# SowpatiLab/ribbit

Hardware: AMD Instinct MI355X
Metric: Gbases/s scanned (m=2..100) (higher is better)
Workload: dtype u32 bit planes

## Files before the change

### ribbit_amd/csrc/api_core.cpp

```cpp
#include "api_internal.h"

#include <sys/mman.h>

namespace rbapi {

thread_local std::string g_last_error;

int fail(int code, const char *fmt, ...) {
    char buf[512];
    va_list ap;
    va_start(ap, fmt);
    vsnprintf(buf, sizeof buf, fmt, ap);
    va_end(ap);
    g_last_error = buf;
    return code;
}


namespace {
constexpr size_t PINNED_HUGE_FROM = (size_t)64 << 20;
std::mutex g_mapped_mu;
std::vector<std::pair<void *, size_t>> g_mapped;
}

// ... 69 lines not shown
int is_gfx950(int device) {
    hipDeviceProp_t prop;
    if (hipGetDeviceProperties(&prop, device) != hipSuccess) return 0;
    return std::strncmp(prop.gcnArchName, "gfx950", 6) == 0;
}

int pack_loaded_ascii(RibbitHandle *h, const uint8_t *dev_ascii, int64_t length) {
    if (h->pair_pending) return fail(RIBBIT_E_STATE, "a perfect scan is in flight on this handle: call ribbit_hip_scan_perfect_end first");
    if (h->copy_pending) { const int rcw = perfect_wait(h); if (rcw) return rcw; }
    h->loaded = false;
    h->dev_ascii_src = dev_ascii;
    h->rec = RibbitHandle::RecordState{};
    if (h->xa_copy_pending) { (void)hipEventSynchronize(h->ev_xa); h->xa_copy_pending = false; }
    h->length = length;
    const int64_t nwords = length / 32 + 1;
    h->ntiles = (nwords + rb::TILE_WORDS - 1) / rb::TILE_WORDS;
    h->tail_words = h->max_shift / 32 + rb::TAIL_SLACK_WORDS;
    h->total_words = rb::LEAD_WORDS + h->ntiles * rb::TILE_WORDS + h->tail_words;
    int rc;
    if ((rc = h->d_hi.ensure((size_t)h->total_words))) return rc;
    if ((rc = h->d_lo.ensure((size_t)h->total_words))) return rc;
    if ((rc = h->d_brk.ensure((size_t)h->total_words))) return rc;
    if (h->timing) HIP_TRY(hipEventRecord(h->timers.begin[RIBBIT_TIME_PACK], h->stream));
    if ((rc = h->pb.d_counters.ensure(rb::EV_COUNTER_WORDS))) return rc;
    rb::launch_pack(dev_ascii, length, h->d_hi.p, h->d_lo.p, h->d_brk.p, h->total_words, h->pb.d_counters.p, rb::EV_COUNTER_WORDS, h->stream);
    h->counters_clean = true;
    HIP_TRY(hipGetLastError());
    if (h->timing) HIP_TRY(hipEventRecord(h->timers.end[RIBBIT_TIME_PACK], h->stream));
    h->timers.have[RIBBIT_TIME_PACK] = h->timing;
    h->lists.perfect.clear(); h->lists.subst.clear(); h->lists.anchored.clear();
    h->lists.range_count = nullptr;
    h->lists.guard_hits = 0;
    h->lists.plane_words = nullptr; h->lists.plane_stride = 0; h->lists.plane_lo = 0; h->lists.plane_hi = -1;
    h->lists.length = length;
    h->lists.min_motif = h->params.min_motif;
    h->lists.max_motif = h->params.max_motif;
    h->lists.min_shift = h->min_shift;
    h->loaded = true;
    return RIBBIT_OK;
}

int ensure_host_planes(RibbitHandle *h) {
    if (h->rec.host_planes_valid) return RIBBIT_OK;
    int rc;
    if ((rc = bind_device(h))) return rc;
    const size_t n = (size_t)(h->ntiles * rb::TILE_WORDS + h->tail_words);
    h->host.resize(h->length, n);
    HIP_TRY(hipMemcpyAsync(h->host.hi.data(), h->d_hi.p + rb::LEAD_WORDS, n * sizeof(uint32_t), hipMemcpyDeviceToHost, h->stream));
    HIP_TRY(hipMemcpyAsync(h->host.lo.data(), h->d_lo.p + rb::LEAD_WORDS, n * sizeof(uint32_t), hipMemcpyDeviceToHost, h->stream));
// ... 283 lines not shown
    } else if (what == RIBBIT_TIME_ANCHORED_PLANES || what == RIBBIT_TIME_ANCHORED_WINDOW) {
        if (!anchored.have_timing || !h->planes_timing_valid) return fail(RIBBIT_E_STATE, "the anchored stage has not run as two kernels on this handle");
        from = what == RIBBIT_TIME_ANCHORED_PLANES ? anchored.ev_begin : h->ev_planes;
        to = what == RIBBIT_TIME_ANCHORED_PLANES ? h->ev_planes : anchored.ev_end;
        last = anchored.ev_end;
    } else {
        if (what < 0 || what > RIBBIT_TIME_ANCHORED_WINDOW) return fail(RIBBIT_E_ARG, "what must be 0..9");
        if (!h->timers.have[what]) return fail(RIBBIT_E_STATE, "no timing recorded yet");
        from = h->timers.begin[what]; to = last = h->timers.end[what];
    }
    float f = 0.f;
    HIP_TRY(hipEventSynchronize(last));
    HIP_TRY(hipEventElapsedTime(&f, from, to));
    *ms = f;
    return RIBBIT_OK;
}); }

int ribbit_hip_debug_stream_read(RibbitHandle *h, int64_t nbytes, int64_t *bytes_read) { return guarded("the stream read", [&]() -> int {
    if (!h || !bytes_read) return fail(RIBBIT_E_ARG, "null argument");
    if (!h->loaded) return fail(RIBBIT_E_STATE, "no record loaded");
    int rc;
    if ((rc = bind_device(h))) return rc;
    if ((rc = h->pb.d_counters.ensure(rb::EV_COUNTER_WORDS))) return rc;
    const uint32_t *src = h->d_events.p ? (const uint32_t *)h->d_events.p : h->d_hi.p;
    const int64_t avail = h->d_events.p ? (int64_t)h->d_events.cap * 8 : h->total_words * 4;
    const int64_t n = std::max<int64_t>(0, std::min(nbytes, avail)) / 4;
    rb::launch_calib_stream_read(src, n, h->pb.d_counters.p + rb::EV_SUMMARY + 8, h->stream);
    HIP_TRY(hipGetLastError());
    HIP_TRY(hipStreamSynchronize(h->stream));
    *bytes_read = n * 4;
    return RIBBIT_OK;
}); }

int64_t ribbit_hip_last_event_count(const RibbitHandle *h) { return h ? h->last_event_count : 0; }

}
```

### ribbit_amd/csrc/api_events.cpp

```cpp
#include "api_internal.h"

namespace rbapi {

int pair_prepare(RibbitHandle *h, PairBufs &pb, int64_t length, int64_t own_lo, int64_t own_hi, int64_t pos_offset, rb::PairLaunch &pr) {
    int rc;
    pr.m_lo = (uint32_t)h->params.min_motif;
    pr.nm = (uint32_t)(h->params.max_motif - h->params.min_motif + 1);
    pr.tile_bases = (uint32_t)rb::TILE_BASES;
    pr.ntile = (uint32_t)(length / rb::TILE_BASES + 1);
    pr.own_lo = own_lo; pr.own_hi = own_hi; pr.pos_offset = pos_offset;
    const size_t entries = (size_t)pr.nm * pr.ntile;
    if (entries > 0xfffffff0u) return fail(RIBBIT_E_ARG, "record too long for %u motif sizes", pr.nm);
    if ((rc = pb.d_counters.ensure(rb::EV_COUNTER_WORDS)) || (rc = pb.d_pair_status.ensure(rb::PAIR_STATUS_WORDS)) ||
        (rc = pb.d_pair_table.ensure(entries)) || (rc = pb.d_run_base.ensure(entries)) || (rc = pb.d_pair_partial.ensure(entries / 1024 + 2)) ||
        (rc = pb.d_halves.ensure(2 * (size_t)pr.nm)))
        return rc;
    if (!pb.h_pub.p) {
        if ((rc = pb.h_pub.ensure(rb::EV_SHARDS + rb::PAIR_STATUS_WORDS))) return rc;
        HIP_TRY(hipHostGetDevicePointer((void **)&pb.h_pub_dev, pb.h_pub.p, 0));
    }
    return RIBBIT_OK;
}

size_t first_event_cap(const RibbitHandle *h, size_t per_base_x4) {
    if (h->debug_first_cap) return h->debug_first_cap;
    return std::max(std::max<size_t>((size_t)1 << 20, (size_t)h->length * per_base_x4 / 4), h->d_events.cap);
}

static size_t round_event_cap(size_t cap) { return std::min<size_t>((cap + rb::EV_SHARDS - 1) / rb::EV_SHARDS * rb::EV_SHARDS, 0xffffff00u); }

int grow_event_cap(int attempt, uint32_t worst, size_t *cap) {
    const size_t need = (size_t)worst * rb::EV_SHARDS;
    if (attempt == 2 || round_event_cap(need) < need) return fail(RIBBIT_E_OVERFLOW, "event buffer overflow: fullest region needs %u events", worst);
    *cap = ((size_t)worst + 1024) * rb::EV_SHARDS;
    return RIBBIT_OK;
}

int event_room(RibbitHandle *h, size_t *cap, rb::PairLaunch *pr) {
    int rc;
    *cap = round_event_cap(*cap);
    if ((rc = h->d_events.ensure(*cap)) || (rc = h->d_dense.ensure(*cap))) return rc;
    if (pr) pr->region_cap = (uint32_t)(*cap / rb::EV_SHARDS);
    return RIBBIT_OK;
}

int zero_counters(RibbitHandle *h, bool even_if_clean) {
    if (even_if_clean || !h->counters_clean) HIP_TRY(hipMemsetAsync(h->pb.d_counters.p, 0, rb::EV_COUNTER_WORDS * sizeof(uint32_t), h->stream));
    h->counters_clean = false;
    return RIBBIT_OK;
}

rb::PerfectLaunch scan_launch_args(const RibbitHandle *h, size_t cap, int kernel) {
    rb::PerfectLaunch pp;
    pp.m_lo = h->params.min_motif;
    pp.m_hi = h->params.max_motif;
    pp.ev_cap = (uint32_t)cap;
    pp.motifs_per_block = h->debug_split[kernel];
    return pp;
}

int enqueue_pairing(PairBufs &pb, const rb::PairLaunch &pr, const uint64_t *d_events, uint64_t *d_dense, size_t cap, hipStream_t stream) {
    HIP_TRY(rb::launch_pair_runs(d_events, pb.d_counters.p, pr, pb.d_pair_table.p, pb.d_run_base.p, pb.d_pair_partial.p,
                                 d_dense, (uint32_t)(cap / 2), pb.d_halves.p, (uint32_t)(2 * (size_t)pr.nm), pb.d_pair_status.p, stream));
    rb::launch_pair_publish(pb.d_counters.p, pb.d_pair_status.p, pb.h_pub_dev, stream);
    HIP_TRY(hipGetLastError());
    return RIBBIT_OK;
}

Published read_published(const PairBufs &pb) {
    Published pub;
    for (int t = 0; t < rb::EV_SHARDS; ++t) { pub.worst = std::max(pub.worst, pb.h_pub.p[t]); pub.produced += pb.h_pub.p[t]; }
    return pub;
}

int pairing_verdict(const PairBufs &pb, uint64_t produced, const char *noun, size_t *n, size_t *n_halves) {
    const uint32_t *status = pb.h_pub.p + rb::EV_SHARDS, flags = status[rb::PAIR_FLAGS];
    if (flags) {
        const std::string s = noun;
        return fail(RIBBIT_E_INTERNAL, "%s pairing failed (flags 0x%x):%s%s%s%s%s", noun, flags,
                    flags & rb::PAIR_BAD_EVENT ? " malformed event;" : "", flags & rb::PAIR_DUP_CHUNK ? " duplicate event chunk;" : "",
                    flags & rb::PAIR_NOT_ALTERNATING ? (" " + s + " starts and ends do not alternate;").c_str() : "",
                    flags & rb::PAIR_UNTERMINATED ? (" unterminated " + s + ";").c_str() : "", flags & rb::PAIR_NO_ROOM ? (" " + s + " buffer too small;").c_str() : "");
    }
    *n = status[rb::PAIR_TOTAL];
    if ((uint64_t)*n * 2 != produced) return fail(RIBBIT_E_INTERNAL, "%llu events but %zu %ss", (unsigned long long)produced, *n, noun);
    *n_halves = status[rb::PAIR_HALVES];
    return RIBBIT_OK;
}

int collect_perfect_events(RibbitHandle *h) {
    int rc;
    if ((rc = bind_device(h))) return rc;
    if ((rc = h->pb.d_counters.ensure(rb::EV_COUNTER_WORDS))) return rc;
    if ((rc = h->h_counters.ensure(rb::EV_COUNTER_WORDS))) return rc;
    size_t cap = first_event_cap(h, 1);
    uint32_t produced = 0;
    for (int attempt = 0;; ++attempt) {
        if ((rc = event_room(h, &cap, nullptr))) return rc;
        HIP_TRY(hipEventRecord(h->timers.begin[RIBBIT_TIME_GPU], h->stream));
        if ((rc = zero_counters(h, true))) return rc;
        const rb::PerfectLaunch pp = scan_launch_args(h, cap, RIBBIT_SCAN_PERFECT);
        HIP_TRY(hipEventRecord(h->timers.begin[RIBBIT_TIME_SCAN], h->stream));
        h->rec.last_split[RIBBIT_SCAN_PERFECT] = rb::launch_scan_perfect(h->planes(), pp, h->d_events.p, h->pb.d_counters.p, h->stream);
        HIP_TRY(hipGetLastError());
        HIP_TRY(hipEventRecord(h->timers.end[RIBBIT_TIME_SCAN], h->stream));
        rb::launch_compact_events(h->d_events.p, pp.ev_cap, h->pb.d_counters.p, h->d_dense.p, h->stream);
        HIP_TRY(hipGetLastError());
        HIP_TRY(hipMemcpyAsync(h->h_counters.p, h->pb.d_counters.p, rb::EV_COUNTER_WORDS * sizeof(uint32_t), hipMemcpyDeviceToHost, h->stream));
        HIP_TRY(hipStreamSynchronize(h->stream));
        produced = h->h_counters.p[rb::EV_SUMMARY];
        if (!h->h_counters.p[rb::EV_SUMMARY + 1]) break;
        uint32_t worst = 0;
        for (int t = 0; t < rb::EV_SHARDS; ++t) worst = std::max(worst, h->h_counters.p[t * rb::EV_COUNTER_STRIDE]);
        if ((rc = grow_event_cap(attempt, worst, &cap))) return rc;
    }
    h->last_event_count = produced;
    if ((rc = h->h_events.ensure(std::max<size_t>(produced, 1)))) return rc;
    const uint32_t m_lo = (uint32_t)h->params.min_motif;
    const size_t nm = (size_t)(h->params.max_motif - h->params.min_motif + 1);
    const size_t ntile = (size_t)(h->length / rb::TILE_BASES + 1);
    if (nm * ntile > 0xfffffff0u) return fail(RIBBIT_E_ARG, "record too long for %zu motif sizes", nm);
    if ((rc = h->pb.d_pair_table.ensure(nm * ntile))) return rc;
    if ((rc = h->pb.d_pair_status.ensure(rb::PAIR_STATUS_WORDS))) return rc;
    HIP_TRY(rb::launch_chunk_table(h->d_dense.p, h->pb.d_counters.p, m_lo, (uint32_t)nm, (uint32_t)ntile, (uint32_t)rb::TILE_BASES, h->pb.d_pair_table.p, h->pb.d_pair_status.p, h->stream));
    h->chunk_table.resize(nm * ntile);
    h->table_ntile = ntile;
    uint32_t table_status = 0;
    HIP_TRY(hipMemcpyAsync(h->chunk_table.data(), h->pb.d_pair_table.p, nm * ntile * sizeof(uint64_t), hipMemcpyDeviceToHost, h->stream));
    HIP_TRY(hipMemcpyAsync(&table_status, h->pb.d_pair_status.p, sizeof(uint32_t), hipMemcpyDeviceToHost, h->stream));
    if (produced) {
        HIP_TRY(hipMemcpyAsync(h->h_events.p, h->d_dense.p, (size_t)produced * sizeof(uint64_t), hipMemcpyDeviceToHost, h->stream));
    }
    HIP_TRY(hipEventRecord(h->timers.end[RIBBIT_TIME_GPU], h->stream));
    HIP_TRY(hipStreamSynchronize(h->stream));
    h->timers.have[RIBBIT_TIME_SCAN] = h->timers.have[RIBBIT_TIME_GPU] = true;
    if (table_status & 1u) return fail(RIBBIT_E_INTERNAL, "malformed event (motif or tile outside the launch)");
    if (table_status & 2u) return fail(RIBBIT_E_INTERNAL, "duplicate event chunk");
    struct Chunk { uint32_t off, n; };
    static_assert(sizeof(Chunk) == sizeof(uint64_t), "chunk table entry is one 64-bit word");
    Chunk *table = reinterpret_cast<Chunk *>(h->chunk_table.data());
    for (size_t k = 0; k < nm * ntile; ++k) {
        const uint32_t first1 = table[k].off, end = table[k].n;
        table[k] = first1 ? Chunk{first1 - 1u, end - (first1 - 1u)} : Chunk{0, 0};
    }
    return RIBBIT_OK;
}

}
```

### ribbit_amd/csrc/api_internal.h

```cpp
#pragma once
#include <hip/hip_runtime_api.h>

#include <algorithm>
#include <atomic>
#include <chrono>
#include <cstdarg>
#include <cstdio>
#include <cstdlib>
#include <condition_variable>
#include <cstring>
#include <deque>
#include <exception>
#include <memory>
#include <mutex>
#include <new>
#include <string>
#include <thread>
#include <vector>

#include "device_planes.h"
#include "event_stream.h"
#include "host_planes.h"
#include "host_threads.h"
#include "kernels.h"
// ... 82 lines not shown
    hipError_t create() { return hipStreamCreateWithFlags(&s, hipStreamNonBlocking); }
    operator hipStream_t() const { return s; }
};
struct OwnedEvent {
    hipEvent_t e = nullptr;
    OwnedEvent() = default;
    OwnedEvent(const OwnedEvent &) = delete;
    OwnedEvent &operator=(const OwnedEvent &) = delete;
    ~OwnedEvent() { if (e) (void)hipEventDestroy(e); }
    hipError_t create(unsigned flags = hipEventDefault) { return hipEventCreateWithFlags(&e, flags); }
    operator hipEvent_t() const { return e; }
};
struct FreeDeleter { void operator()(void *p) const { std::free(p); } };

inline double now_ms() {
    using namespace std::chrono;
    return duration<double, std::milli>(steady_clock::now().time_since_epoch()).count();
}

enum Stage { STAGE_NONE = 0, STAGE_PERFECT = 1, STAGE_SUBST = 2, STAGE_ANCHORED = 3 };

struct PairBufs {
    DevBuf<uint32_t> d_counters;
    DevBuf<uint64_t> d_pair_table;
    DevBuf<uint32_t> d_run_base, d_pair_partial, d_pair_status;
    DevBuf<RibbitRun> d_halves;
    PinnedBuf<uint32_t> h_pub;
    uint32_t *h_pub_dev = nullptr;
};


template <typename T>
int hand_out(const T *src, size_t n, bool terminate, T **out) {
    T *mem = static_cast<T *>(std::malloc((std::max<size_t>(n, 1) + (terminate ? 1 : 0)) * sizeof(T)));
    if (!mem) return fail(RIBBIT_E_NOMEM, "out of host memory");
    if (src && n) std::memcpy(mem, src, n * sizeof(T));
    if (terminate) mem[n] = T();
    *out = mem;
    return RIBBIT_OK;
}

struct ClippedRow { int64_t s, e; size_t index; };
inline std::vector<ClippedRow> clipped_sorted_rows(int64_t length, const int32_t *intervals, size_t n) {
    std::vector<ClippedRow> rows;
    rows.reserve(n);
    for (size_t i = 0; i < n; ++i) {
        const int64_t s = std::max<int64_t>(intervals[2 * i], 0), e = std::min<int64_t>(intervals[2 * i + 1], length);
        if (s < e) rows.push_back(ClippedRow{s, e, i});
    }
    std::sort(rows.begin(), rows.end(), [](const ClippedRow &a, const ClippedRow &b) { return a.s != b.s ? a.s < b.s : a.index < b.index; });
    return rows;
// ... 52 lines not shown
    DevBuf<uint8_t> d_ascii;
    DevBuf<uint32_t> d_hi, d_lo, d_brk;
    DevBuf<uint64_t> d_events, d_dense;
    DevBuf<uint32_t> d_query;
    DevBuf<uint32_t> d_xa;
    int64_t xa_stride = 0;
    PinnedBuf<uint64_t> h_events;
    PinnedBuf<uint32_t> h_counters;
    PinnedBuf<uint32_t> h_query;

    rb::HostPlanes host;

    int64_t last_event_count = 0;
    std::vector<uint64_t> chunk_table;
    size_t table_ntile = 0;

    std::vector<RibbitRun> runs;
    PairBufs pb;
    PinnedBuf<RibbitRun> h_runs, h_halves;
    rb::PairLaunch pair{};
    bool pair_pending = false;
    size_t debug_first_cap = 0;
    int32_t debug_split[RIBBIT_SCAN_KERNELS] = {};
    bool counters_clean = false;
    bool copy_pending = false;
    size_t n_runs = 0, n_halves = 0;
    DevBuf<uint32_t> d_eval, d_first_rev, d_word_tmp, d_last_word, d_bitmap, d_edge_tmp, d_edge_end1, d_ws_counters;
    DevBuf<uint64_t> d_group, d_sort_keys, d_sort_vals, d_edge_keys, d_edge_vals, d_edge_keys2, d_edge_vals2;
    DevBuf<int32_t> d_min_span, d_pend, d_tj;
    DevBuf<uint32_t> d_dropmap;
    bool dropmap_valid = false;
    DevBuf<RibbitCall> d_flush;
    DevBuf<uint8_t> d_scratch;
    struct WindowStage {
        PinnedBuf<RibbitCall> h_calls, h_flush;
        PinnedBuf<int32_t> h_pend;
        PinnedBuf<uint32_t> h_ws;
        OwnedEvent ev_begin, ev_end;
        bool have_timing = false;
    } win[3];
    PinnedBuf<uint32_t> h_xa;
    struct MergeBufs {
        DevBuf<RibbitSeed> d_perfect, d_subst, d_own;
        DevBuf<int32_t> d_type0, d_cuts;
        DevBuf<uint32_t> d_first, d_range_out, d_log, d_head_log, d_counts, d_scratch;
        PinnedBuf<RibbitSeed> h_own;
        PinnedBuf<uint32_t> h_range_out, h_log, h_head_log, h_counts, h_sync;
// ... 85 lines not shown

namespace rbapi {


using DeviceCalls = rb::KeptCalls;


struct ChunkWindow {
    uint32_t own_lo = 0, own_hi = 0xffffffffu, z_lo = 0;
    bool keep_flush = true;
    int32_t pos_offset = 0;
    bool inexact = false;
};

int bind_device(const RibbitHandle *h);
int is_gfx950(int device);
int pack_loaded_ascii(RibbitHandle *h, const uint8_t *dev_ascii, int64_t length);
int ensure_host_planes(RibbitHandle *h);
inline size_t dropmap_words(int64_t length) { return (size_t)(length / 32 + 1) + 1024; }
int pair_prepare(RibbitHandle *h, PairBufs &pb, int64_t length, int64_t own_lo, int64_t own_hi, int64_t pos_offset, rb::PairLaunch &pr);
size_t first_event_cap(const RibbitHandle *h, size_t per_base_x4);
int grow_event_cap(int attempt, uint32_t worst, size_t *cap);
int event_room(RibbitHandle *h, size_t *cap, rb::PairLaunch *pr);
int zero_counters(RibbitHandle *h, bool even_if_clean = false);
rb::PerfectLaunch scan_launch_args(const RibbitHandle *h, size_t cap, int kernel);
int enqueue_pairing(PairBufs &pb, const rb::PairLaunch &pr, const uint64_t *d_events, uint64_t *d_dense, size_t cap, hipStream_t stream);
struct Published { uint32_t worst = 0; uint64_t produced = 0; };
Published read_published(const PairBufs &pb);
int pairing_verdict(const PairBufs &pb, uint64_t produced, const char *noun, size_t *n, size_t *n_halves);
int collect_perfect_events(RibbitHandle *h);
rb::EventSource event_source(const RibbitHandle *h);
int perfect_wait(RibbitHandle *h);
int perfect_enqueue(RibbitHandle *h, size_t cap);
int perfect_begin(RibbitHandle *h, int64_t own_lo, int64_t own_hi, int64_t pos_offset);
int perfect_collect(RibbitHandle *h);
int perfect_finish(RibbitHandle *h, RibbitRun *dst, size_t dst_cap, RibbitRun *half_dst, size_t half_dst_cap, bool wait = true);
int run_perfect_scan_range(RibbitHandle *h, int64_t own_lo, int64_t own_hi, int64_t pos_offset, RibbitRun *dst, size_t dst_cap,
                           RibbitRun *half_dst = nullptr, size_t half_dst_cap = 0);
int run_perfect_scan(RibbitHandle *h);
int build_perfect_calls(RibbitHandle *h);
int advance_to_perfect(RibbitHandle *h);
int scan_and_pair_streaks(RibbitHandle *h, int stage , uint32_t *n_streaks, int (*filter_min_span)(int) = nullptr);
int window_stage_device(RibbitHandle *h, int stage, bool full, int (*min_span)(int), DeviceCalls *out, ChunkWindow *cw = nullptr);
void full_calls_from_device(const DeviceCalls &dc, rb::CallVec &calls);
int build_subst_calls(RibbitHandle *h);
void subst_merge(RibbitHandle *h, const DeviceCalls *dc);
// ... 27 lines not shown
```

### ribbit_amd/csrc/api_perfect.cpp

```cpp
#include "api_internal.h"

namespace rbapi {

rb::EventSource event_source(const RibbitHandle *h) {
    rb::EventSource src;
    src.ev = h->h_events.p;
    src.segs = reinterpret_cast<const rb::Seg *>(h->chunk_table.data());
    src.segs_per_motif = h->table_ntile;
    src.nm = (size_t)(h->params.max_motif - h->params.min_motif + 1);
    src.m_lo = h->params.min_motif;
    return src;
}

int perfect_wait(RibbitHandle *h) {
    if (!h->copy_pending) return RIBBIT_OK;
    h->copy_pending = false;
    int rc;
    if ((rc = bind_device(h))) return rc;
    HIP_TRY(hipStreamSynchronize(h->copy_stream));
    return RIBBIT_OK;
}

int perfect_enqueue(RibbitHandle *h, size_t cap) {
    int rc;
// ... 202 lines not shown
    if (!h || !out || !n) return fail(RIBBIT_E_ARG, "null argument");
    int rc = perfect_finish(h, dst, dst_cap, half_dst, half_dst_cap, wait != 0);
    if (rc) return rc;
    *out = dst ? dst : h->h_runs.p;
    *n = h->n_runs;
    if (halves) *halves = half_dst ? half_dst : h->h_halves.p;
    if (n_halves) *n_halves = h->n_halves;
    return RIBBIT_OK;
}); }

int ribbit_hip_debug_pair_events(RibbitHandle *h, const uint64_t *events, size_t n, int64_t length, RibbitRun *runs, size_t runs_cap,
                                 size_t *n_runs, uint32_t *flags) { return guarded("the pairing of the events", [&]() -> int {
    if (!h || (n && !events) || !n_runs || !flags || (runs_cap && !runs)) return fail(RIBBIT_E_ARG, "null argument");
    if (length < 0 || n > ((size_t)1 << 24)) return fail(RIBBIT_E_ARG, "bad size");
    int rc;
    if ((rc = bind_device(h))) return rc;
    rb::PairLaunch pr{};
    PairBufs pb;
    if ((rc = pair_prepare(h, pb, length, 0, INT64_MAX, 0, pr))) return rc;
    pr.region_cap = (uint32_t)std::max<size_t>(n, 1);
    const size_t cap = (size_t)pr.region_cap * rb::EV_SHARDS;
    DevBuf<uint64_t> d_ev, d_runs;
    if ((rc = d_ev.ensure(cap)) || (rc = d_runs.ensure(cap))) return rc;
    std::vector<uint32_t> counters(rb::EV_COUNTER_WORDS, 0);
    counters[0] = (uint32_t)n;
    if (n) HIP_TRY(hipMemcpy(d_ev.p, events, n * sizeof(uint64_t), hipMemcpyHostToDevice));
    HIP_TRY(hipMemcpy(pb.d_counters.p, counters.data(), counters.size() * sizeof(uint32_t), hipMemcpyHostToDevice));
    if ((rc = enqueue_pairing(pb, pr, d_ev.p, d_runs.p, cap, h->stream))) return rc;
    HIP_TRY(hipStreamSynchronize(h->stream));
    const uint32_t *status = pb.h_pub.p + rb::EV_SHARDS;
    *flags = status[rb::PAIR_FLAGS];
    *n_runs = status[rb::PAIR_TOTAL];
    const size_t take = std::min(*n_runs, runs_cap);
    if (take) HIP_TRY(hipMemcpy(runs, d_runs.p, take * sizeof(RibbitRun), hipMemcpyDeviceToHost));
    return RIBBIT_OK;
}); }

int ribbit_host_perfect_runs_from_events(const RibbitScanParams *params, size_t nparts, const uint64_t *events,
                                         const uint64_t *counts, RibbitRun **runs, size_t *n) { return guarded("the pairing of the events", [&]() -> int {
    if (!params || !counts || !runs || !n) return fail(RIBBIT_E_ARG, "null argument");
    const size_t nm = (size_t)(params->max_motif - params->min_motif + 1);
    std::vector<rb::Seg> segs(nm * nparts, rb::Seg{0, 0});
    uint64_t off = 0;
    for (size_t p = 0; p < nparts; ++p)
        for (size_t mi = 0; mi < nm; ++mi) { segs[mi * nparts + p] = rb::Seg{(uint32_t)off, (uint32_t)counts[p * nm + mi]}; off += counts[p * nm + mi]; }
    rb::EventSource src;
    src.ev = events; src.segs = segs.data(); src.segs_per_motif = nparts; src.nm = nm; src.m_lo = params->min_motif;
// ... 14 lines not shown
```

### ribbit_amd/csrc/device_planes.h

```cpp
#pragma once
#include <stdint.h>

namespace rb {

constexpr int WORDS_PER_LANE = 8;
constexpr int TILE_WORDS = 64 * WORDS_PER_LANE;
constexpr int TILE_BASES = TILE_WORDS * 32;
constexpr int LEAD_WORDS = 72;
constexpr int TAIL_SLACK_WORDS = 544;

struct DevicePlanes {
    const uint32_t *hi;
    const uint32_t *lo;
    const uint32_t *brk;
    int64_t length;
    int64_t ntiles;
    int64_t tail_words;
};

constexpr int ANCHORED_MAX_MOTIF = 990;
__host__ __device__ inline int anchored_halo_lanes(int max_motif) { return (2 * (max_motif + 2) + 32 + 255) / 256; }
__host__ __device__ inline int anchored_tile_words(int hl) { return (64 - 2 * hl) * WORDS_PER_LANE; }

constexpr int EV_SHARDS = 64;
constexpr int EV_COUNTER_STRIDE = 32;
constexpr int EV_SUMMARY = EV_SHARDS * EV_COUNTER_STRIDE;
constexpr int EV_COUNTER_WORDS = EV_SUMMARY + EV_COUNTER_STRIDE;

enum : uint32_t { EV_START = 0, EV_END_ZERO = 1, EV_END_N = 2, EV_END_EOS = 3 };

__host__ __device__ inline uint64_t ev_pack(uint32_t pos, uint32_t mlen, uint32_t kind) {
    return (uint64_t)pos | ((uint64_t)mlen << 32) | ((uint64_t)kind << 48);
}
__host__ __device__ inline uint32_t ev_pos(uint64_t e) { return (uint32_t)e; }
__host__ __device__ inline uint32_t ev_mlen(uint64_t e) { return (uint32_t)(e >> 32) & 0xffffu; }
__host__ __device__ inline uint32_t ev_kind(uint64_t e) { return (uint32_t)(e >> 48) & 0xfu; }

enum : int32_t { RUN_NOT_OWNED = -1, RUN_HALF_START = 3, RUN_HALF_END = 4  };

enum : uint32_t { PAIR_FLAGS = 0, PAIR_TOTAL = 1, PAIR_HALVES = 2, PAIR_STATUS_WORDS = 4 };
enum : uint32_t {
    PAIR_BAD_EVENT = 1,
    PAIR_DUP_CHUNK = 2,
    PAIR_NOT_ALTERNATING = 4,
    PAIR_UNTERMINATED = 8,
    PAIR_NO_ROOM = 16,
};

}
```

### ribbit_amd/csrc/kernels.h

```cpp
#pragma once
#include <hip/hip_runtime_api.h>
#include <stdint.h>

#include <algorithm>

#include "device_planes.h"
#include "ribbit_hip.h"

namespace rb {

void launch_pack(const uint8_t *dev_ascii, int64_t length, uint32_t *hi, uint32_t *lo, uint32_t *brk,
                 int64_t total_words, uint32_t *zero_words, int n_zero, hipStream_t stream);

struct PerfectLaunch {
    int m_lo, m_hi;
    uint32_t ev_cap;
    int motifs_per_block = 0;
};
struct ScanSplit {
    int grid_y = 0, motifs_per_block = 0;
};
ScanSplit launch_scan_perfect(const DevicePlanes &pl, const PerfectLaunch &pp, uint64_t *events, uint32_t *counters,
                              hipStream_t stream);

ScanSplit launch_scan_window(const DevicePlanes &pl, const PerfectLaunch &pp, int allowed_mismatches, uint64_t *events,
                             uint32_t *counters, hipStream_t stream);

ScanSplit launch_scan_anchored(const DevicePlanes &pl, const PerfectLaunch &pp, uint32_t *xa, int64_t xa_stride, hipStream_t stream);
constexpr int GROUP_FILTER_MAX = 16;
ScanSplit launch_scan_xa_window(const DevicePlanes &pl, const PerfectLaunch &pp, const uint32_t *xa, int64_t xa_stride, uint64_t *events,
                                uint32_t *counters, const int32_t *tj_table, uint32_t *dropmap, hipStream_t stream);

void launch_compact_events(const uint64_t *events, uint32_t ev_cap, uint32_t *counters, uint64_t *dense,
                           hipStream_t stream);

struct PairLaunch {
    uint32_t m_lo, nm;
    uint32_t ntile;
    uint32_t tile_bases;
    uint32_t region_cap;
    int64_t own_lo, own_hi, pos_offset;
};
hipError_t launch_pair_runs(const uint64_t *events, const uint32_t *counters, const PairLaunch &pl, void *table,
                            uint32_t *run_base, uint32_t *partial, void *runs, uint32_t run_cap, void *halves,
                            uint32_t half_cap, uint32_t *status, hipStream_t stream);

void launch_pair_publish(const uint32_t *counters, const uint32_t *status, uint32_t *host_words, hipStream_t stream);

hipError_t launch_chunk_table(const uint64_t *dense, const uint32_t *counters, uint32_t m_lo, uint32_t nm, uint32_t ntile,
                              uint32_t tile_bases, void *table, uint32_t *status, hipStream_t stream);

enum : uint32_t { WS_N_MAIN = 0, WS_N_EDGE = 1, WS_FLAGS = 2, WS_MAX_END = 3 ,
                  WS_INEXACT = 4 , WS_WORDS = 8 };
enum : uint32_t {
    WS_TWO_FLUSH = 1,
    WS_BAD_MOTIF = 2,
    WS_NOT_PROMPT = 4,
    WS_EDGE_LOST = 8,
};
hipError_t launch_eval_planes(const uint32_t *brk, uint32_t n_words, uint32_t *eval, uint32_t *first_rev, uint32_t *word_tmp,
                              void *scratch, size_t scratch_bytes, hipStream_t stream);
hipError_t launch_group_starts(const RibbitRun *runs, uint32_t n, uint32_t m_lo, uint64_t *group, void *scratch,
                               size_t scratch_bytes, hipStream_t stream);
struct WindowCallsLaunch {
    const RibbitRun *runs; uint32_t n_streaks;
    const uint64_t *group;
    const uint32_t *eval, *first_rev, *brk; uint32_t n_words;
    int64_t length;
    uint32_t m_lo, nm;
    const int32_t *min_span;
// ... 127 lines not shown
```

### ribbit_amd/csrc/kernels.hip

```cpp
#include <hip/hip_runtime.h>

#include <algorithm>
#include <climits>
#include <type_traits>

#include "kernels.h"

namespace rb {

__device__ __forceinline__ uint32_t funnel(uint32_t hi, uint32_t lo, uint32_t sh) {
    return __builtin_amdgcn_alignbit(hi, lo, sh);
}

template <unsigned TT>
__device__ __forceinline__ uint32_t bitop3(uint32_t a, uint32_t b, uint32_t c) {
    return __builtin_amdgcn_bitop3_b32(a, b, c, TT);
}

__global__ __launch_bounds__(256) void pack_kernel(const uint8_t *__restrict__ ascii, int64_t length,
                                                   uint32_t *__restrict__ hi, uint32_t *__restrict__ lo,
                                                   uint32_t *__restrict__ brk, int64_t total_words,
                                                   uint32_t *__restrict__ zero_words, int n_zero) {
    const int64_t t = (int64_t)blockIdx.x * blockDim.x + threadIdx.x;
    if (blockIdx.x == 0)
// ... 1079 lines not shown
    for (uint32_t i = blockIdx.x * 256u + threadIdx.x; i < n; i += gridDim.x * 256u) {
        const uint64_t e = ev[i];
        uint32_t key, other;
        if (!chunk_key_of(e, pl, key)) { atomicOr(&status[PAIR_FLAGS], (uint32_t)PAIR_BAD_EVENT); continue; }
        const uint32_t g = shard * pl.region_cap + i;
        const bool first = i == 0 || !chunk_key_of(ev[i - 1], pl, other) || other != key;
        const bool last = i + 1 == n || !chunk_key_of(ev[i + 1], pl, other) || other != key;
        if (first && atomicExch(&table[key].begin1, g + 1u) != 0u) atomicOr(&status[PAIR_FLAGS], (uint32_t)PAIR_DUP_CHUNK);
        if (last) table[key].end1 = g + 2u;
        if (!first && (ev_kind(ev[i - 1]) == EV_START) == (ev_kind(e) == EV_START))
            atomicOr(&status[PAIR_FLAGS], (uint32_t)PAIR_NOT_ALTERNATING);
    }
}

__device__ __forceinline__ uint32_t chunk_start_count(const ChunkEntry *table, const uint64_t *events, uint32_t key) {
    const ChunkEntry c = table[key];
    if (c.begin1 == 0u) return 0u;
    const uint32_t cnt = c.end1 - c.begin1;
    return (cnt + (ev_kind(events[c.begin1 - 1u]) == EV_START ? 1u : 0u)) >> 1;
}

constexpr int SCAN_ITEMS = 4;
constexpr int SCAN_BLOCK = 256 * SCAN_ITEMS;

__device__ __forceinline__ uint32_t block_exclusive_scan(uint32_t v, uint32_t &block_total) {
    __shared__ uint32_t wave_sum[4];
    const int lane = threadIdx.x & 63, wave = threadIdx.x >> 6;
    const uint32_t incl = (uint32_t)wave_inclusive_scan((int)v);
    if (lane == 63) wave_sum[wave] = incl;
    __syncthreads();
    uint32_t before = 0, total = 0;
#pragma unroll
    for (int w = 0; w < 4; w++) { if (w < wave) before += wave_sum[w]; total += wave_sum[w]; }
    __syncthreads();
    block_total = total;
    return before + incl - v;
}

__global__ __launch_bounds__(256) void pair_chunk_starts_kernel(const ChunkEntry *__restrict__ table,
                                                                const uint64_t *__restrict__ events, uint32_t entries,
                                                                uint32_t *__restrict__ run_base,
                                                                uint32_t *__restrict__ partial) {
    const uint32_t base = blockIdx.x * (uint32_t)SCAN_BLOCK + threadIdx.x * (uint32_t)SCAN_ITEMS;
    uint32_t sum = 0;
#pragma unroll
    for (int k = 0; k < SCAN_ITEMS; k++) {
        const uint32_t key = base + (uint32_t)k;
        const uint32_t c = key < entries ? chunk_start_count(table, events, key) : 0u;
        if (key < entries) run_base[key] = c;
        sum += c;
    }
    uint32_t total;
    (void)block_exclusive_scan(sum, total);
    if (threadIdx.x == 0) partial[blockIdx.x] = total;
}

__global__ __launch_bounds__(256) void pair_scan_partials_kernel(uint32_t *__restrict__ partial, uint32_t nblocks,
                                                                 uint32_t *__restrict__ status) {
    uint32_t carry = 0;
    for (uint32_t base = 0; base < nblocks; base += 256u) {
        const uint32_t i = base + threadIdx.x;
        const uint32_t v = i < nblocks ? partial[i] : 0u;
        uint32_t total;
        const uint32_t excl = block_exclusive_scan(v, total);
        if (i < nblocks) partial[i] = carry + excl;
        carry += total;
    }
    if (threadIdx.x == 0) status[PAIR_TOTAL] = carry;
}

__global__ __launch_bounds__(256) void pair_run_base_kernel(uint32_t entries, const uint32_t *__restrict__ partial,
                                                            uint32_t *__restrict__ run_base) {
    const uint32_t base = blockIdx.x * (uint32_t)SCAN_BLOCK + threadIdx.x * (uint32_t)SCAN_ITEMS;
    uint32_t c[SCAN_ITEMS], sum = 0;
#pragma unroll
    for (int k = 0; k < SCAN_ITEMS; k++) {
        c[k] = base + (uint32_t)k < entries ? run_base[base + (uint32_t)k] : 0u;
        sum += c[k];
    }
    uint32_t total;
    uint32_t at = partial[blockIdx.x] + block_exclusive_scan(sum, total);
#pragma unroll
    for (int k = 0; k < SCAN_ITEMS; k++) {
        if (base + (uint32_t)k < entries) run_base[base + (uint32_t)k] = at;
        at += c[k];
    }
}

struct RunRecord { int32_t start, end, mlen, term; };

__global__ __launch_bounds__(256) void pair_runs_kernel(const uint64_t *__restrict__ events,
                                                        const uint32_t *__restrict__ counters, PairLaunch pl,
                                                        const ChunkEntry *__restrict__ table,
                                                        const uint32_t *__restrict__ run_base,
                                                        RunRecord *__restrict__ runs, uint32_t run_cap,
                                                        RunRecord *__restrict__ halves, uint32_t half_cap,
                                                        uint32_t *__restrict__ status) {
    const uint32_t shard = blockIdx.y;
    const uint32_t n = region_count(counters, shard, pl.region_cap);
    const uint64_t *ev = events + (size_t)shard * pl.region_cap;
    for (uint32_t i = blockIdx.x * 256u + threadIdx.x; i < n; i += gridDim.x * 256u) {
        const uint64_t e = ev[i];
        uint32_t key;
        if (!chunk_key_of(e, pl, key)) continue;
        const ChunkEntry c = table[key];
        const uint32_t g1 = shard * pl.region_cap + i + 1u;
        if (c.begin1 == 0u || g1 < c.begin1 || g1 >= c.end1) continue;
        const uint32_t mi = key / pl.ntile, tile = key - mi * pl.ntile;
        const bool chunk_opens_with_end = ev_kind(events[c.begin1 - 1u]) != EV_START;
        if (ev_kind(e) != EV_START) {
            if (g1 == c.begin1) {
                bool ok = false;
                for (uint32_t t = tile; t-- > 0u;) {
                    const ChunkEntry p = table[mi * pl.ntile + t];
                    if (p.begin1 == 0u) continue;
                    ok = ev_kind(events[p.end1 - 2u]) == EV_START;
                    break;
                }
                if (!ok) atomicOr(&status[PAIR_FLAGS], (uint32_t)PAIR_NOT_ALTERNATING);
            }
// ... 11 lines not shown
                break;
            }
        }
        if (!found) { atomicOr(&status[PAIR_FLAGS], (uint32_t)PAIR_UNTERMINATED); continue; }
        const uint32_t kind = ev_kind(closer);
        if (kind == EV_START || ev_pos(closer) <= ev_pos(e)) { atomicOr(&status[PAIR_FLAGS], (uint32_t)PAIR_NOT_ALTERNATING); continue; }
        const uint32_t in_chunk = (g1 - c.begin1 - (chunk_opens_with_end ? 1u : 0u)) >> 1;
        const uint32_t slot = run_base[key] + in_chunk;
        if (slot >= run_cap) { atomicOr(&status[PAIR_FLAGS], (uint32_t)PAIR_NO_ROOM); continue; }
        const int64_t rs = (int64_t)ev_pos(e), re = (int64_t)ev_pos(closer);
        const int32_t mlen = (int32_t)(mi + pl.m_lo), term = (int32_t)kind - 1;
        const bool start_owned = rs >= pl.own_lo && rs < pl.own_hi, end_owned = re >= pl.own_lo && re < pl.own_hi;
        if (start_owned && re < pl.own_hi) {
            runs[slot] = RunRecord{(int32_t)(rs + pl.pos_offset), (int32_t)(re + pl.pos_offset), mlen, term};
            continue;
        }
        runs[slot] = RunRecord{0, 0, 0, RUN_NOT_OWNED};
        if (!start_owned && !end_owned) continue;
        const uint32_t at = atomicAdd(&status[PAIR_HALVES], 1u);
        if (at >= half_cap) { atomicOr(&status[PAIR_FLAGS], (uint32_t)PAIR_NO_ROOM); continue; }
        halves[at] = start_owned ? RunRecord{(int32_t)(rs + pl.pos_offset), -1, mlen, RUN_HALF_START}
                                 : RunRecord{-1, (int32_t)(re + pl.pos_offset), mlen, RUN_HALF_END + term};
    }
}

__global__ __launch_bounds__(128) void pair_publish_kernel(const uint32_t *__restrict__ counters,
                                                           const uint32_t *__restrict__ status,
                                                           uint32_t *__restrict__ host_words) {
    const uint32_t t = threadIdx.x;
    if (t < (uint32_t)EV_SHARDS) host_words[t] = counters[t * EV_COUNTER_STRIDE];
    else if (t < (uint32_t)EV_SHARDS + PAIR_STATUS_WORDS) host_words[t] = status[t - (uint32_t)EV_SHARDS];
    __threadfence_system();
}

void launch_pair_publish(const uint32_t *counters, const uint32_t *status, uint32_t *host_words, hipStream_t stream) {
    hipLaunchKernelGGL(pair_publish_kernel, dim3(1), dim3(128), 0, stream, counters, status, host_words);
}

hipError_t launch_pair_runs(const uint64_t *events, const uint32_t *counters, const PairLaunch &pl, void *table,
                            uint32_t *run_base, uint32_t *partial, void *runs, uint32_t run_cap, void *halves,
                            uint32_t half_cap, uint32_t *status, hipStream_t stream) {
    const uint32_t entries = pl.nm * pl.ntile;
    const uint32_t nblocks = (entries + (uint32_t)SCAN_BLOCK - 1u) / (uint32_t)SCAN_BLOCK;
    const uint32_t per_region = std::min<uint32_t>(std::max<uint32_t>((pl.region_cap + 255u) / 256u, 1u), 64u);
    hipError_t e = hipMemsetAsync(table, 0, (size_t)entries * sizeof(ChunkEntry), stream);
    if (e != hipSuccess) return e;
    if ((e = hipMemsetAsync(status, 0, PAIR_STATUS_WORDS * sizeof(uint32_t), stream)) != hipSuccess) return e;
    hipLaunchKernelGGL(pair_chunk_bounds_kernel, dim3(per_region, EV_SHARDS), dim3(256), 0, stream, events, counters, pl,
                       (ChunkEntry *)table, status);
    hipLaunchKernelGGL(pair_chunk_starts_kernel, dim3(nblocks), dim3(256), 0, stream, (const ChunkEntry *)table, events,
                       entries, run_base, partial);
    hipLaunchKernelGGL(pair_scan_partials_kernel, dim3(1), dim3(256), 0, stream, partial, nblocks, status);
    hipLaunchKernelGGL(pair_run_base_kernel, dim3(nblocks), dim3(256), 0, stream, entries, (const uint32_t *)partial, run_base);
    hipLaunchKernelGGL(pair_runs_kernel, dim3(per_region, EV_SHARDS), dim3(256), 0, stream, events, counters, pl,
                       (const ChunkEntry *)table, (const uint32_t *)run_base, (RunRecord *)runs, run_cap,
                       (RunRecord *)halves, half_cap, status);
    return hipGetLastError();
}

__global__ __launch_bounds__(256) void plane_words_kernel(DevicePlanes pl, int shift, int64_t w0, int64_t nw,
                                                          uint32_t *__restrict__ out_words, int64_t p0, int64_t p1,
                                                          uint32_t *__restrict__ count) {
    const int64_t i = (int64_t)blockIdx.x * blockDim.x + threadIdx.x;
    uint32_t bits = 0;
    if (i < nw) {
        const int64_t w = w0 + i;
        const int q = shift >> 5;
        const uint32_t r = (uint32_t)shift & 31u;
        const uint32_t hs = funnel(pl.hi[w + q + 1], pl.hi[w + q], r);
        const uint32_t ls = funnel(pl.lo[w + q + 1], pl.lo[w + q], r);
        const uint32_t x = ~((pl.hi[w] ^ hs) | (pl.lo[w] ^ ls));
        if (out_words) out_words[i] = x;
        if (count) {
            const int64_t lo_p = w * 32, hi_p = lo_p + 32;
            uint32_t mask = 0xffffffffu;
            if (p0 > lo_p) mask &= (p0 >= hi_p) ? 0u : (0xffffffffu << (uint32_t)(p0 - lo_p));
            if (p1 < hi_p) mask &= (p1 <= lo_p) ? 0u : (0xffffffffu >> (uint32_t)(hi_p - p1));
            bits = (uint32_t)__popc(x & mask);
        }
// ... 172 lines not shown
```

Before: 432.0.

## Fuse pairing prefix scan into single-pass decoupled look-back kernel and fold publish

Replaces the three-kernel prefix sum over chunk run counts (count, scan partials in one block, add offsets) with a single decoupled look-back scan using dynamic block tickets. The host publish kernel is folded into the runs kernel through a last-block ticket. Pair status and look-back state now live after the counters buffer, so the status memset joins the counter zeroing that pack already does. This aims to cut kernel launches, memsets and the serial single-block scan, at the cost of spin-wait look-back and atomics.

```diff
diff --git a/ribbit_amd/csrc/api_core.cpp b/ribbit_amd/csrc/api_core.cpp
--- a/ribbit_amd/csrc/api_core.cpp
+++ b/ribbit_amd/csrc/api_core.cpp
@@ -115,9 +115,11 @@
     if ((rc = h->d_lo.ensure((size_t)h->total_words))) return rc;
     if ((rc = h->d_brk.ensure((size_t)h->total_words))) return rc;
     if (h->timing) HIP_TRY(hipEventRecord(h->timers.begin[RIBBIT_TIME_PACK], h->stream));
-    if ((rc = h->pb.d_counters.ensure(rb::EV_COUNTER_WORDS))) return rc;
-    rb::launch_pack(dev_ascii, length, h->d_hi.p, h->d_lo.p, h->d_brk.p, h->total_words, h->pb.d_counters.p, rb::EV_COUNTER_WORDS, h->stream);
-    h->counters_clean = true;
+    const size_t entries = pair_entries(h, length);
+    if ((rc = h->pb.ensure_words(entries))) return rc;
+    const size_t n_zero = PairBufs::words_for(entries) <= ((size_t)1 << 16) ? PairBufs::words_for(entries) : (size_t)rb::EV_COUNTER_WORDS;
+    rb::launch_pack(dev_ascii, length, h->d_hi.p, h->d_lo.p, h->d_brk.p, h->total_words, h->pb.d_counters.p, (int)n_zero, h->stream);
+    h->pb.clean_words = n_zero;
     HIP_TRY(hipGetLastError());
     if (h->timing) HIP_TRY(hipEventRecord(h->timers.end[RIBBIT_TIME_PACK], h->stream));
     h->timers.have[RIBBIT_TIME_PACK] = h->timing;
@@ -447,6 +449,7 @@
     int rc;
     if ((rc = bind_device(h))) return rc;
     if ((rc = h->pb.d_counters.ensure(rb::EV_COUNTER_WORDS))) return rc;
+    h->pb.clean_words = 0;
     const uint32_t *src = h->d_events.p ? (const uint32_t *)h->d_events.p : h->d_hi.p;
     const int64_t avail = h->d_events.p ? (int64_t)h->d_events.cap * 8 : h->total_words * 4;
     const int64_t n = std::max<int64_t>(0, std::min(nbytes, avail)) / 4;
diff --git a/ribbit_amd/csrc/api_events.cpp b/ribbit_amd/csrc/api_events.cpp
--- a/ribbit_amd/csrc/api_events.cpp
+++ b/ribbit_amd/csrc/api_events.cpp
@@ -1,6 +1,10 @@
 #include "api_internal.h"
 
 namespace rbapi {
+
+size_t pair_entries(const RibbitHandle *h, int64_t length) {
+    return (size_t)(h->params.max_motif - h->params.min_motif + 1) * (size_t)(length / rb::TILE_BASES + 1);
+}
 
 int pair_prepare(RibbitHandle *h, PairBufs &pb, int64_t length, int64_t own_lo, int64_t own_hi, int64_t pos_offset, rb::PairLaunch &pr) {
     int rc;
@@ -9,10 +13,9 @@
     pr.tile_bases = (uint32_t)rb::TILE_BASES;
     pr.ntile = (uint32_t)(length / rb::TILE_BASES + 1);
     pr.own_lo = own_lo; pr.own_hi = own_hi; pr.pos_offset = pos_offset;
-    const size_t entries = (size_t)pr.nm * pr.ntile;
+    const size_t entries = pair_entries(h, length);
     if (entries > 0xfffffff0u) return fail(RIBBIT_E_ARG, "record too long for %u motif sizes", pr.nm);
-    if ((rc = pb.d_counters.ensure(rb::EV_COUNTER_WORDS)) || (rc = pb.d_pair_status.ensure(rb::PAIR_STATUS_WORDS)) ||
-        (rc = pb.d_pair_table.ensure(entries)) || (rc = pb.d_run_base.ensure(entries)) || (rc = pb.d_pair_partial.ensure(entries / 1024 + 2)) ||
+    if ((rc = pb.ensure_words(entries)) || (rc = pb.d_pair_table.ensure(entries)) || (rc = pb.d_run_base.ensure(entries)) ||
         (rc = pb.d_halves.ensure(2 * (size_t)pr.nm)))
         return rc;
     if (!pb.h_pub.p) {
@@ -45,8 +48,13 @@
 }
 
 int zero_counters(RibbitHandle *h, bool even_if_clean) {
-    if (even_if_clean || !h->counters_clean) HIP_TRY(hipMemsetAsync(h->pb.d_counters.p, 0, rb::EV_COUNTER_WORDS * sizeof(uint32_t), h->stream));
-    h->counters_clean = false;
+    PairBufs &pb = h->pb;
+    const size_t entries = pair_entries(h, h->length);
+    int rc;
+    if ((rc = pb.ensure_words(entries))) return rc;
+    const size_t need = PairBufs::words_for(entries);
+    if (even_if_clean || pb.clean_words < need) HIP_TRY(hipMemsetAsync(pb.d_counters.p, 0, need * sizeof(uint32_t), h->stream));
+    pb.clean_words = 0;
     return RIBBIT_OK;
 }
 
@@ -60,10 +68,9 @@
 }
 
 int enqueue_pairing(PairBufs &pb, const rb::PairLaunch &pr, const uint64_t *d_events, uint64_t *d_dense, size_t cap, hipStream_t stream) {
-    HIP_TRY(rb::launch_pair_runs(d_events, pb.d_counters.p, pr, pb.d_pair_table.p, pb.d_run_base.p, pb.d_pair_partial.p,
-                                 d_dense, (uint32_t)(cap / 2), pb.d_halves.p, (uint32_t)(2 * (size_t)pr.nm), pb.d_pair_status.p, stream));
-    rb::launch_pair_publish(pb.d_counters.p, pb.d_pair_status.p, pb.h_pub_dev, stream);
-    HIP_TRY(hipGetLastError());
+    pb.clean_words = 0;
+    HIP_TRY(rb::launch_pair_runs(d_events, pb.d_counters.p, pr, pb.d_pair_table.p, pb.d_run_base.p, d_dense, (uint32_t)(cap / 2),
+                                 pb.d_halves.p, (uint32_t)(2 * (size_t)pr.nm), pb.state(), pb.h_pub_dev, stream));
     return RIBBIT_OK;
 }
 
@@ -91,7 +98,6 @@
 int collect_perfect_events(RibbitHandle *h) {
     int rc;
     if ((rc = bind_device(h))) return rc;
-    if ((rc = h->pb.d_counters.ensure(rb::EV_COUNTER_WORDS))) return rc;
     if ((rc = h->h_counters.ensure(rb::EV_COUNTER_WORDS))) return rc;
     size_t cap = first_event_cap(h, 1);
     uint32_t produced = 0;
@@ -121,13 +127,13 @@
     const size_t ntile = (size_t)(h->length / rb::TILE_BASES + 1);
     if (nm * ntile > 0xfffffff0u) return fail(RIBBIT_E_ARG, "record too long for %zu motif sizes", nm);
     if ((rc = h->pb.d_pair_table.ensure(nm * ntile))) return rc;
-    if ((rc = h->pb.d_pair_status.ensure(rb::PAIR_STATUS_WORDS))) return rc;
-    HIP_TRY(rb::launch_chunk_table(h->d_dense.p, h->pb.d_counters.p, m_lo, (uint32_t)nm, (uint32_t)ntile, (uint32_t)rb::TILE_BASES, h->pb.d_pair_table.p, h->pb.d_pair_status.p, h->stream));
+    if ((rc = h->pb.d_table_status.ensure(1))) return rc;
+    HIP_TRY(rb::launch_chunk_table(h->d_dense.p, h->pb.d_counters.p, m_lo, (uint32_t)nm, (uint32_t)ntile, (uint32_t)rb::TILE_BASES, h->pb.d_pair_table.p, h->pb.d_table_status.p, h->stream));
     h->chunk_table.resize(nm * ntile);
     h->table_ntile = ntile;
     uint32_t table_status = 0;
     HIP_TRY(hipMemcpyAsync(h->chunk_table.data(), h->pb.d_pair_table.p, nm * ntile * sizeof(uint64_t), hipMemcpyDeviceToHost, h->stream));
-    HIP_TRY(hipMemcpyAsync(&table_status, h->pb.d_pair_status.p, sizeof(uint32_t), hipMemcpyDeviceToHost, h->stream));
+    HIP_TRY(hipMemcpyAsync(&table_status, h->pb.d_table_status.p, sizeof(uint32_t), hipMemcpyDeviceToHost, h->stream));
     if (produced) {
         HIP_TRY(hipMemcpyAsync(h->h_events.p, h->d_dense.p, (size_t)produced * sizeof(uint64_t), hipMemcpyDeviceToHost, h->stream));
     }
diff --git a/ribbit_amd/csrc/api_internal.h b/ribbit_amd/csrc/api_internal.h
--- a/ribbit_amd/csrc/api_internal.h
+++ b/ribbit_amd/csrc/api_internal.h
@@ -128,11 +128,20 @@
 
 struct PairBufs {
     DevBuf<uint32_t> d_counters;
+    size_t clean_words = 0;
     DevBuf<uint64_t> d_pair_table;
-    DevBuf<uint32_t> d_run_base, d_pair_partial, d_pair_status;
+    DevBuf<uint32_t> d_run_base;
+    DevBuf<uint32_t> d_table_status;
     DevBuf<RibbitRun> d_halves;
     PinnedBuf<uint32_t> h_pub;
     uint32_t *h_pub_dev = nullptr;
+
+    static size_t words_for(size_t entries) { return rb::EV_COUNTER_WORDS + rb::pair_state_words(entries); }
+    int ensure_words(size_t entries) {
+        if (words_for(entries) > d_counters.cap) clean_words = 0;
+        return d_counters.ensure(words_for(entries));
+    }
+    uint32_t *state() const { return d_counters.p + rb::EV_COUNTER_WORDS; }
 };
 
 
@@ -231,7 +240,6 @@
     bool pair_pending = false;
     size_t debug_first_cap = 0;
     int32_t debug_split[RIBBIT_SCAN_KERNELS] = {};
-    bool counters_clean = false;
     bool copy_pending = false;
     size_t n_runs = 0, n_halves = 0;
     DevBuf<uint32_t> d_eval, d_first_rev, d_word_tmp, d_last_word, d_bitmap, d_edge_tmp, d_edge_end1, d_ws_counters;
@@ -363,6 +371,7 @@
 size_t first_event_cap(const RibbitHandle *h, size_t per_base_x4);
 int grow_event_cap(int attempt, uint32_t worst, size_t *cap);
 int event_room(RibbitHandle *h, size_t *cap, rb::PairLaunch *pr);
+size_t pair_entries(const RibbitHandle *h, int64_t length);
 int zero_counters(RibbitHandle *h, bool even_if_clean = false);
 rb::PerfectLaunch scan_launch_args(const RibbitHandle *h, size_t cap, int kernel);
 int enqueue_pairing(PairBufs &pb, const rb::PairLaunch &pr, const uint64_t *d_events, uint64_t *d_dense, size_t cap, hipStream_t stream);
diff --git a/ribbit_amd/csrc/api_perfect.cpp b/ribbit_amd/csrc/api_perfect.cpp
--- a/ribbit_amd/csrc/api_perfect.cpp
+++ b/ribbit_amd/csrc/api_perfect.cpp
@@ -248,7 +248,7 @@
     const size_t cap = (size_t)pr.region_cap * rb::EV_SHARDS;
     DevBuf<uint64_t> d_ev, d_runs;
     if ((rc = d_ev.ensure(cap)) || (rc = d_runs.ensure(cap))) return rc;
-    std::vector<uint32_t> counters(rb::EV_COUNTER_WORDS, 0);
+    std::vector<uint32_t> counters(PairBufs::words_for(pair_entries(h, length)), 0);
     counters[0] = (uint32_t)n;
     if (n) HIP_TRY(hipMemcpy(d_ev.p, events, n * sizeof(uint64_t), hipMemcpyHostToDevice));
     HIP_TRY(hipMemcpy(pb.d_counters.p, counters.data(), counters.size() * sizeof(uint32_t), hipMemcpyHostToDevice));
diff --git a/ribbit_amd/csrc/device_planes.h b/ribbit_amd/csrc/device_planes.h
--- a/ribbit_amd/csrc/device_planes.h
+++ b/ribbit_amd/csrc/device_planes.h
@@ -1,4 +1,5 @@
 #pragma once
+#include <stddef.h>
 #include <stdint.h>
 
 namespace rb {
@@ -38,7 +39,10 @@
 
 enum : int32_t { RUN_NOT_OWNED = -1, RUN_HALF_START = 3, RUN_HALF_END = 4  };
 
-enum : uint32_t { PAIR_FLAGS = 0, PAIR_TOTAL = 1, PAIR_HALVES = 2, PAIR_STATUS_WORDS = 4 };
+enum : uint32_t { PAIR_FLAGS = 0, PAIR_TOTAL = 1, PAIR_HALVES = 2, PAIR_RUNS_TICKET = 3, PAIR_STATUS_WORDS = 4 };
+constexpr uint32_t PAIR_PREFIX_TICKET = 4, PAIR_LOOK_WORDS = 8, PAIR_PREFIX_BLOCK = 1024;
+__host__ __device__ inline size_t pair_prefix_blocks(size_t entries) { return (entries + PAIR_PREFIX_BLOCK - 1) / PAIR_PREFIX_BLOCK; }
+__host__ __device__ inline size_t pair_state_words(size_t entries) { return PAIR_LOOK_WORDS + 2 * pair_prefix_blocks(entries); }
 enum : uint32_t {
     PAIR_BAD_EVENT = 1,
     PAIR_DUP_CHUNK = 2,
diff --git a/ribbit_amd/csrc/kernels.h b/ribbit_amd/csrc/kernels.h
--- a/ribbit_amd/csrc/kernels.h
+++ b/ribbit_amd/csrc/kernels.h
@@ -42,10 +42,8 @@
     int64_t own_lo, own_hi, pos_offset;
 };
 hipError_t launch_pair_runs(const uint64_t *events, const uint32_t *counters, const PairLaunch &pl, void *table,
-                            uint32_t *run_base, uint32_t *partial, void *runs, uint32_t run_cap, void *halves,
-                            uint32_t half_cap, uint32_t *status, hipStream_t stream);
-
-void launch_pair_publish(const uint32_t *counters, const uint32_t *status, uint32_t *host_words, hipStream_t stream);
+                            uint32_t *run_base, void *runs, uint32_t run_cap, void *halves, uint32_t half_cap,
+                            uint32_t *state, uint32_t *host_words, hipStream_t stream);
 
 hipError_t launch_chunk_table(const uint64_t *dense, const uint32_t *counters, uint32_t m_lo, uint32_t nm, uint32_t ntile,
                               uint32_t tile_bases, void *table, uint32_t *status, hipStream_t stream);
diff --git a/ribbit_amd/csrc/kernels.hip b/ribbit_amd/csrc/kernels.hip
--- a/ribbit_amd/csrc/kernels.hip
+++ b/ribbit_amd/csrc/kernels.hip
@@ -1125,6 +1125,7 @@
 
 constexpr int SCAN_ITEMS = 4;
 constexpr int SCAN_BLOCK = 256 * SCAN_ITEMS;
+static_assert(SCAN_BLOCK == (int)PAIR_PREFIX_BLOCK, "one look-back word per block of the prefix kernel");
 
 __device__ __forceinline__ uint32_t block_exclusive_scan(uint32_t v, uint32_t &block_total) {
     __shared__ uint32_t wave_sum[4];
@@ -1140,49 +1141,53 @@
     return before + incl - v;
 }
 
-__global__ __launch_bounds__(256) void pair_chunk_starts_kernel(const ChunkEntry *__restrict__ table,
-                                                                const uint64_t *__restrict__ events, uint32_t entries,
-                                                                uint32_t *__restrict__ run_base,
-                                                                uint32_t *__restrict__ partial) {
-    const uint32_t base = blockIdx.x * (uint32_t)SCAN_BLOCK + threadIdx.x * (uint32_t)SCAN_ITEMS;
-    uint32_t sum = 0;
+constexpr unsigned long long LOOK_AGGREGATE = 1ull << 32, LOOK_INCLUSIVE = 2ull << 32;
+
+__global__ __launch_bounds__(256) void pair_prefix_kernel(const ChunkEntry *__restrict__ table,
+                                                          const uint64_t *__restrict__ events, uint32_t entries,
+                                                          uint32_t nblocks, uint32_t *__restrict__ run_base,
+                                                          uint32_t *__restrict__ ticket,
+                                                          unsigned long long *__restrict__ look,
+                                                          uint32_t *__restrict__ status) {
+    __shared__ uint32_t s_block, s_carry;
+    if (threadIdx.x == 0) s_block = atomicAdd(ticket, 1u);
+    __syncthreads();
+    const uint32_t block = s_block;
+    if (block >= nblocks) return;
+    const uint32_t base = block * (uint32_t)SCAN_BLOCK + threadIdx.x * (uint32_t)SCAN_ITEMS;
+    uint32_t c[SCAN_ITEMS], sum = 0;
 #pragma unroll
     for (int k = 0; k < SCAN_ITEMS; k++) {
         const uint32_t key = base + (uint32_t)k;
-        const uint32_t c = key < entries ? chunk_start_count(table, events, key) : 0u;
-        if (key < entries) run_base[key] = c;
-        sum += c;
+        c[k] = key < entries ? chunk_start_count(table, events, key) : 0u;
+        sum += c[k];
     }
     uint32_t total;
-    (void)block_exclusive_scan(sum, total);
-    if (threadIdx.x == 0) partial[blockIdx.x] = total;
-}
-
-__global__ __launch_bounds__(256) void pair_scan_partials_kernel(uint32_t *__restrict__ partial, uint32_t nblocks,
-                                                                 uint32_t *__restrict__ status) {
-    uint32_t carry = 0;
-    for (uint32_t base = 0; base < nblocks; base += 256u) {
-        const uint32_t i = base + threadIdx.x;
-        const uint32_t v = i < nblocks ? partial[i] : 0u;
-        uint32_t total;
-        const uint32_t excl = block_exclusive_scan(v, total);
-        if (i < nblocks) partial[i] = carry + excl;
-        carry += total;
-    }
-    if (threadIdx.x == 0) status[PAIR_TOTAL] = carry;
-}
-
-__global__ __launch_bounds__(256) void pair_run_base_kernel(uint32_t entries, const uint32_t *__restrict__ partial,
-                                                            uint32_t *__restrict__ run_base) {
-    const uint32_t base = blockIdx.x * (uint32_t)SCAN_BLOCK + threadIdx.x * (uint32_t)SCAN_ITEMS;
-    uint32_t c[SCAN_ITEMS], sum = 0;
-#pragma unroll
-    for (int k = 0; k < SCAN_ITEMS; k++) {
-        c[k] = base + (uint32_t)k < entries ? run_base[base + (uint32_t)k] : 0u;
-        sum += c[k];
-    }
-    uint32_t total;
-    uint32_t at = partial[blockIdx.x] + block_exclusive_scan(sum, total);
+    const uint32_t excl = block_exclusive_scan(sum, total);
+    if (threadIdx.x < 64u) {
+        const uint32_t lane = threadIdx.x;
+        if (lane == 0 && block != 0u)
+            __hip_atomic_store(&look[block], LOOK_AGGREGATE | total, __ATOMIC_RELAXED, __HIP_MEMORY_SCOPE_AGENT);
+        uint32_t carry = 0;
+        for (int64_t first = (int64_t)block - 1;; first -= 64) {
+            const int64_t at = first - (int64_t)lane;
+            unsigned long long w = LOOK_INCLUSIVE;
+            if (at >= 0)
+                do w = __hip_atomic_load(&look[at], __ATOMIC_RELAXED, __HIP_MEMORY_SCOPE_AGENT); while ((w >> 32) == 0ull);
+            const unsigned long long inclusive = __ballot((w >> 32) == 2ull);
+            const uint32_t stop = inclusive ? (uint32_t)__ffsll((long long)inclusive) - 1u : 63u;
+            const uint32_t upto = (uint32_t)wave_inclusive_scan((int)(lane <= stop ? (uint32_t)w : 0u));
+            carry += (uint32_t)__shfl((int)upto, 63);
+            if (inclusive) break;
+        }
+        if (lane == 0) {
+            __hip_atomic_store(&look[block], LOOK_INCLUSIVE | (carry + total), __ATOMIC_RELAXED, __HIP_MEMORY_SCOPE_AGENT);
+            if (block + 1u == nblocks) status[PAIR_TOTAL] = carry + total;
+            s_carry = carry;
+        }
+    }
+    __syncthreads();
+    uint32_t at = s_carry + excl;
 #pragma unroll
     for (int k = 0; k < SCAN_ITEMS; k++) {
         if (base + (uint32_t)k < entries) run_base[base + (uint32_t)k] = at;
@@ -1198,7 +1203,8 @@
                                                         const uint32_t *__restrict__ run_base,
                                                         RunRecord *__restrict__ runs, uint32_t run_cap,
                                                         RunRecord *__restrict__ halves, uint32_t half_cap,
-                                                        uint32_t *__restrict__ status) {
+                                                        uint32_t *__restrict__ status,
+                                                        uint32_t *__restrict__ host_words) {
     const uint32_t shard = blockIdx.y;
     const uint32_t n = region_count(counters, shard, pl.region_cap);
     const uint64_t *ev = events + (size_t)shard * pl.region_cap;
@@ -1256,39 +1262,37 @@
         halves[at] = start_owned ? RunRecord{(int32_t)(rs + pl.pos_offset), -1, mlen, RUN_HALF_START}
                                  : RunRecord{-1, (int32_t)(re + pl.pos_offset), mlen, RUN_HALF_END + term};
     }
-}
-
-__global__ __launch_bounds__(128) void pair_publish_kernel(const uint32_t *__restrict__ counters,
-                                                           const uint32_t *__restrict__ status,
-                                                           uint32_t *__restrict__ host_words) {
+    __shared__ uint32_t s_last;
+    __threadfence();
+    __syncthreads();
+    if (threadIdx.x == 0) s_last = atomicAdd(&status[PAIR_RUNS_TICKET], 1u) + 1u == gridDim.x * gridDim.y ? 1u : 0u;
+    __syncthreads();
+    if (!s_last) return;
+    __threadfence();
     const uint32_t t = threadIdx.x;
     if (t < (uint32_t)EV_SHARDS) host_words[t] = counters[t * EV_COUNTER_STRIDE];
-    else if (t < (uint32_t)EV_SHARDS + PAIR_STATUS_WORDS) host_words[t] = status[t - (uint32_t)EV_SHARDS];
+    else if (t < (uint32_t)EV_SHARDS + PAIR_STATUS_WORDS) {
+        const uint32_t w = t - (uint32_t)EV_SHARDS;
+        host_words[t] = w == PAIR_RUNS_TICKET ? 0u : __hip_atomic_load(&status[w], __ATOMIC_RELAXED, __HIP_MEMORY_SCOPE_AGENT);
+    }
     __threadfence_system();
 }
 
-void launch_pair_publish(const uint32_t *counters, const uint32_t *status, uint32_t *host_words, hipStream_t stream) {
-    hipLaunchKernelGGL(pair_publish_kernel, dim3(1), dim3(128), 0, stream, counters, status, host_words);
-}
-
 hipError_t launch_pair_runs(const uint64_t *events, const uint32_t *counters, const PairLaunch &pl, void *table,
-                            uint32_t *run_base, uint32_t *partial, void *runs, uint32_t run_cap, void *halves,
-                            uint32_t half_cap, uint32_t *status, hipStream_t stream) {
+                            uint32_t *run_base, void *runs, uint32_t run_cap, void *halves, uint32_t half_cap,
+                            uint32_t *state, uint32_t *host_words, hipStream_t stream) {
     const uint32_t entries = pl.nm * pl.ntile;
-    const uint32_t nblocks = (entries + (uint32_t)SCAN_BLOCK - 1u) / (uint32_t)SCAN_BLOCK;
+    const uint32_t nblocks = (uint32_t)pair_prefix_blocks(entries);
     const uint32_t per_region = std::min<uint32_t>(std::max<uint32_t>((pl.region_cap + 255u) / 256u, 1u), 64u);
     hipError_t e = hipMemsetAsync(table, 0, (size_t)entries * sizeof(ChunkEntry), stream);
     if (e != hipSuccess) return e;
-    if ((e = hipMemsetAsync(status, 0, PAIR_STATUS_WORDS * sizeof(uint32_t), stream)) != hipSuccess) return e;
     hipLaunchKernelGGL(pair_chunk_bounds_kernel, dim3(per_region, EV_SHARDS), dim3(256), 0, stream, events, counters, pl,
-                       (ChunkEntry *)table, status);
-    hipLaunchKernelGGL(pair_chunk_starts_kernel, dim3(nblocks), dim3(256), 0, stream, (const ChunkEntry *)table, events,
-                       entries, run_base, partial);
-    hipLaunchKernelGGL(pair_scan_partials_kernel, dim3(1), dim3(256), 0, stream, partial, nblocks, status);
-    hipLaunchKernelGGL(pair_run_base_kernel, dim3(nblocks), dim3(256), 0, stream, entries, (const uint32_t *)partial, run_base);
+                       (ChunkEntry *)table, state);
+    hipLaunchKernelGGL(pair_prefix_kernel, dim3(nblocks), dim3(256), 0, stream, (const ChunkEntry *)table, events, entries,
+                       nblocks, run_base, state + PAIR_PREFIX_TICKET, (unsigned long long *)(state + PAIR_LOOK_WORDS), state);
     hipLaunchKernelGGL(pair_runs_kernel, dim3(per_region, EV_SHARDS), dim3(256), 0, stream, events, counters, pl,
                        (const ChunkEntry *)table, (const uint32_t *)run_base, (RunRecord *)runs, run_cap,
-                       (RunRecord *)halves, half_cap, status);
+                       (RunRecord *)halves, half_cap, state, host_words);
     return hipGetLastError();
 }
 
```

Measured after the change: 157.6. 0.365x the previous value.
